# Human-Augment-Analytics/vectordb-retrieval

Hardware: AMD Instinct MI355X
Metric: QPS @ recall@10 (SIFT1M-shaped, 10k-query batch, k=10) (higher is better)
Workload: dtype i8 MFMA scan (i32 accumulate) + exact integer / f64 refine

## Files before the change

vectordb-retrieval_amd/csrc/scan_i8x16.hpp:

```cpp
#pragma once
#include "scan_i8.hpp"

namespace vdb {

__host__ __device__ inline int x16_row_in_span(int t, int rb, int m) { return (m >> 2) * 128 + t * 8 + rb * 4 + (m & 3); }

__device__ __forceinline__ int swap16(int v) { return __builtin_amdgcn_ds_swizzle(v, 0x401F); }

template <int KS2, int ST, int RING>
constexpr int scan_i8x16_lds_bytes() { return RING * (ST * 2 * KS2 * 64 * 16 + ST * 32 * 4); }

template <int N_MFMA, int N_VALU, int N_DS>
__device__ __forceinline__ void x16_gap_pattern() {
    constexpr int R = (N_VALU + N_DS + N_MFMA - 1) / N_MFMA;
    static_assert(N_DS <= N_MFMA && R >= 2, "one LDS read per gap");
#pragma unroll
    for (int i = 0; i < N_MFMA; ++i) {
        __builtin_amdgcn_sched_group_barrier(0x8, 1, 0);
        if (i < N_DS) {
            __builtin_amdgcn_sched_group_barrier(0x100, 1, 0);
            __builtin_amdgcn_sched_group_barrier(0x2, R - 1, 0);
        } else {
            __builtin_amdgcn_sched_group_barrier(0x2, R, 0);
        }
    }
}

template <int KS2, int ST, int CB, class StageIssue, class BiasStore, class FlushBin>
__device__ __forceinline__ void scan_i8x16_batch_loop(const unsigned char *smem, const int4v (&bq)[CB][KS2], int (&m1)[CB], int (&m2)[CB],
                                                      int nstages, int64_t span0, int lane, StageIssue &&stage_issue,
                                                      BiasStore &&stage_bias_store, FlushBin &&flush_bin) {
    constexpr int NV = 2 * KS2, kStageVec = ST * NV * 64, TPS = kTilesPerSpan, SPS = TPS / ST;
    constexpr int NM = 2 * KS2 * CB, NH = NM / 2;
    static_assert(ST % 2 == 0 && TPS % ST == 0, "tile parity must be static in the unrolled stage");
    const int g = lane >> 4;
    const unsigned id_hi = (g & 1) ? 16u : 0u;
    int4v acc[2][2][CB], fr[2][NV], cin[2][2];
    int q[CB];
#pragma unroll
    for (int rb = 0; rb < 2; ++rb)
#pragma unroll
        for (int cb = 0; cb < CB; ++cb)
#pragma unroll
            for (int r = 0; r < 4; ++r) acc[1][rb][cb][r] = (int)(kI8Inf >> 6);
    auto read_tile = [&](int p, const int4v *A, const int4v *B4, int t) {
#pragma unroll
        for (int v = 0; v < NV; ++v) fr[p][v] = A[(t * NV + v) * 64];
        cin[p][0] = B4[t * 8];
        cin[p][1] = B4[t * 8 + 1];
    };
    auto mfma_half = [&](int p, int half) {
#pragma unroll
        for (int m = half * NH; m < (half + 1) * NH; ++m) {
            const int ks = m / (2 * CB), rb = (m / CB) % 2, cb = m % CB;
            acc[p][rb][cb] = __builtin_amdgcn_mfma_i32_16x16x64_i8(fr[p][2 * ks + rb], bq[cb][ks], ks == 0 ? cin[p][rb] : acc[p][rb][cb], 0, 0, 0);
        }
    };
    auto min_trees = [&](int o) {
#pragma unroll
        for (int cb = 0; cb < CB; ++cb) {
            const int t1 = imin(imin(acc[o][0][cb][0], acc[o][0][cb][1]), acc[o][0][cb][2]);
            const int t2 = imin(imin(acc[o][0][cb][3], acc[o][1][cb][0]), acc[o][1][cb][1]);
            q[cb] = imin(imin(imin(acc[o][1][cb][2], acc[o][1][cb][3]), t1), t2);
        }
    };
    auto folds = [&](int t_bin) {
        const unsigned idv = (unsigned)__builtin_amdgcn_readfirstlane(t_bin) | id_hi;
#pragma unroll
        for (int cb = 0; cb < CB; ++cb) {
            const int v = (int)(((unsigned)q[cb] << 6) | idv);
            m2[cb] = imed3(m1[cb], m2[cb], v);
            m1[cb] = imin(m1[cb], v);
        }
    };
    for (int st = 0; st < nstages; ++st) {
        const int buf = st & 1;
        if (st + 1 < nstages) stage_issue(st + 1, buf ^ 1);
        const int4v *A = reinterpret_cast<const int4v *>(smem + buf * (kStageVec * 16)) + lane;
        const int4v *B4 = reinterpret_cast<const int4v *>(smem + 2 * kStageVec * 16 + buf * (ST * 32 * 4)) + g * 2;
        const int ts0 = (st % SPS) * ST;
        read_tile(0, A, B4, 0);
#pragma unroll
        for (int t = 0; t < ST; ++t) {
            const int p = t & 1, o = p ^ 1;
            __builtin_amdgcn_sched_barrier(0);
            mfma_half(p, 0);
            min_trees(o);
            x16_gap_pattern<NH, 4 * CB, 0>();
            __builtin_amdgcn_sched_barrier(0);
#pragma unroll
            for (int cb = 0; cb < CB; ++cb) asm volatile("" : "+v"(q[cb]));
            __builtin_amdgcn_sched_barrier(0);
            if (t + 1 < ST) read_tile(o, A, B4, t + 1);
            mfma_half(p, 1);
            folds((ts0 + t + TPS - 1) % TPS);
            x16_gap_pattern<NH, 3 * CB + 1, NV + 2>();
            __builtin_amdgcn_sched_barrier(0);
#pragma unroll
            for (int cb = 0; cb < CB; ++cb) asm volatile("" : "+v"(m1[cb]), "+v"(m2[cb]));
            if (t == 0 && st > 0 && ts0 == 0) flush_bin(span0 + st / SPS - 1);
        }
        __builtin_amdgcn_sched_barrier(0);
        if (st + 1 < nstages) stage_bias_store(buf ^ 1);
        __syncthreads();
    }
    min_trees((ST - 1) & 1);
    folds(TPS - 1);
    flush_bin(span0 + nstages / SPS - 1);
}

template <int KS2, int ST, int CB, int NWAVES = 8, int RING = 2, int AUX = 0>
__device__ __forceinline__ void scan_i8x16_body(const ScanI8Args &a, unsigned char *smem) {
    constexpr int NV = 2 * KS2;
    constexpr int NT = NWAVES * 64;
    constexpr int kStageVec = ST * NV * 64;
    constexpr int kBiasLoads = (ST * 32 + NT - 1) / NT;
    constexpr int TPS = kTilesPerSpan;
    constexpr int SPS = TPS / ST;
    constexpr int HC = CB / 2;
    constexpr int UNR = (ST * CB <= 16) ? ST : 1;
    static_assert(TPS % ST == 0 && ST >= 2 && CB % 2 == 0 && NWAVES <= 8, "bad geometry");
    static_assert(RING >= 2 && RING <= 8 && (RING == 2 || ST % 2 == 0), "bad ring");
    constexpr bool kDeep = RING > 2;
    static_assert(scan_i8x16_lds_bytes<KS2, ST, RING>() == RING * (kStageVec * 16 + ST * 32 * 4), "LDS size");
    const int mode = a.info->i8_mode;
    if (!mode) return;
    auto lds_a = [&](int buf) { return reinterpret_cast<int4v *>(smem + buf * (kStageVec * 16)); };
    auto lds_b = [&](int buf) { return reinterpret_cast<int *>(smem + RING * kStageVec * 16 + buf * (ST * 32 * 4)); };

    const int tid = threadIdx.x, lane = tid & 63;
    const int wave = __builtin_amdgcn_readfirstlane(tid >> 6);
    const int g = lane >> 4, h = g >> 1;
    const bool odd = (g & 1) != 0;
    const bool late = (NWAVES >= 2) && (wave >= NWAVES / 2);
    const int b = blockIdx.x;
    const int x = b & 7, jb = b >> 3;
    const int ci = jb / a.nqtiles, qt = jb - ci * a.nqtiles;
    const int chunk = x + 8 * ci;
    if (chunk >= a.nchunks) return;
    const int64_t q0 = (int64_t)qt * (NWAVES * 16 * CB) + wave * (16 * CB);
    const int64_t span0 = chunk_span0(chunk, a.spans_per_chunk, a.chunk_rem);
    int64_t span1 = chunk_span0(chunk + 1, a.spans_per_chunk, a.chunk_rem);
    if (span1 > a.nspans) span1 = a.nspans;
    const int64_t out_pitch = a.Qpad;
    const int64_t col0 = q0 + (odd ? 16 : 0) + (lane & 15);
    const int32_t *bias = a.bias8 + ((mode & 3) == 1 ? 0 : a.Npad);

    int4v bq[CB][KS2];
#pragma unroll
    for (int cb = 0; cb < CB; ++cb)
#pragma unroll
        for (int ks = 0; ks < KS2; ++ks) bq[cb][ks] = a.qpanels[((size_t)(q0 / 16 + cb) * KS2 + ks) * 64 + lane];
    const int nstages = (int)(span1 - span0) * SPS;
    const int INF = (int)kI8Inf;
    int m1[CB], m2[CB], M1[HC], M2[HC], Ms[HC];
#pragma unroll
    for (int cb = 0; cb < CB; ++cb) m1[cb] = m2[cb] = INF;
#pragma unroll
    for (int j = 0; j < HC; ++j) {
        M1[j] = M2[j] = INF;
        Ms[j] = 0;
    }

    constexpr int kPieces = kStageVec / 64;
    static_assert(kPieces % NWAVES == 0, "pieces must divide over the waves");
    constexpr int kBiasPieces = (ST / 2 + NWAVES - 1) / NWAVES;
    int stage_b[kBiasLoads];
    auto stage_issue = [&](int st, int buf) {
        const int64_t span = span0 + st / SPS;
        const int sq = st % SPS;
        const int4v *src = a.panels + ((size_t)(span * TPS + sq * ST) * NV) * 64;
        int4v *dst = lds_a(buf);
#pragma unroll
        for (int i = 0; i < kPieces / NWAVES; ++i) {
            const int p = wave + i * NWAVES;
            const int4v *gp = src + p * 64 + lane;
            __builtin_amdgcn_global_load_lds(
                reinterpret_cast<const __attribute__((address_space(1))) void *>(reinterpret_cast<uintptr_t>(gp)),
                reinterpret_cast<__attribute__((address_space(3))) void *>(
                    static_cast<uint32_t>(reinterpret_cast<uintptr_t>(dst + p * 64))),
                16, 0, AUX);
        }
        if (kDeep) {
#pragma unroll
            for (int i = 0; i < kBiasPieces; ++i) {
                const int j = (wave + i * NWAVES) % (ST / 2);
                const int t = 2 * j + (lane >> 5), gg = (lane >> 3) & 3, e = lane & 7;
                const int32_t *gp = bias + span * kSpanRows + gg * 128 + (sq * ST + t) * 8 + e;
                __builtin_amdgcn_global_load_lds(
                    reinterpret_cast<const __attribute__((address_space(1))) void *>(reinterpret_cast<uintptr_t>(gp)),
                    reinterpret_cast<__attribute__((address_space(3))) void *>(
                        static_cast<uint32_t>(reinterpret_cast<uintptr_t>(lds_b(buf) + j * 64))),
                    4, 0, 0);
            }
            return;
        }
#pragma unroll
        for (int i = 0; i < kBiasLoads; ++i) {
            const int e = tid + i * NT;
            if (e < ST * 32) {
                const int t = e >> 5, gg = (e >> 3) & 3, r = e & 7;
                stage_b[i] = bias[span * kSpanRows + gg * 128 + (sq * ST + t) * 8 + r];
            }
        }
    };
    auto stage_bias_store = [&](int buf) {
        if (kDeep) return;
#pragma unroll
        for (int i = 0; i < kBiasLoads; ++i)
            if (tid + i * NT < ST * 32) lds_b(buf)[tid + i * NT] = stage_b[i];
    };
    auto ring_issue = [&](int st) { stage_issue(st < nstages ? st : nstages - 1, st % RING); };
    auto ring_wait = [&]() {
        constexpr int kKeep = (RING - 2) * (kPieces / NWAVES + kBiasPieces);
        static_assert(kKeep < 64, "vmcnt is a 6-bit counter");
        asm volatile("s_waitcnt vmcnt(%0)" ::"n"(kKeep) : "memory");
        __builtin_amdgcn_s_barrier();
        asm volatile("" ::: "memory");
    };
    auto flush_bin = [&](int64_t span) {
        const size_t o = (size_t)(span * 2 + h) * out_pitch + col0;
#pragma unroll
        for (int j = 0; j < HC; ++j) {
            const int p1 = swap16(odd ? m1[2 * j] : m1[2 * j + 1]), p2 = swap16(odd ? m2[2 * j] : m2[2 * j + 1]);
            const int a1 = odd ? m1[2 * j + 1] : m1[2 * j], a2 = odd ? m2[2 * j + 1] : m2[2 * j];
            const int b1 = imin(a1, p1), b2 = imin(imax(a1, p1), imin(a2, p2));
            __builtin_nontemporal_store(__int_as_float(b1), a.bin_m1 + o + j * 32);
            __builtin_nontemporal_store(__int_as_float(b2), a.bin_m2 + o + j * 32);
            M2[j] = imin(imed3(M1[j], M2[j], b1), b2);
            if (b1 < M1[j]) Ms[j] = (int)span;
            M1[j] = imin(M1[j], b1);
        }
#pragma unroll
        for (int cb = 0; cb < CB; ++cb) m1[cb] = m2[cb] = INF;
    };

    if (kDeep) {
#pragma unroll
        for (int s = 0; s < RING - 1; ++s) ring_issue(s);
    } else {
        stage_issue(0, 0);
    }
    stage_bias_store(0);
    if (kDeep) ring_wait();
    else __syncthreads();

    if (a.nq_valid > 0 && q0 >= a.nq_valid) {
        for (int st = 0; st < nstages; ++st) {
            if (kDeep) {
                ring_issue(st + RING - 1);
                ring_wait();
                continue;
            }
            if (st + 1 < nstages) {
                stage_issue(st + 1, (st & 1) ^ 1);
                stage_bias_store((st & 1) ^ 1);
            }
            __syncthreads();
        }
        return;
    }

    if constexpr (NWAVES == 8 && RING == 2 && UNR == 1) {
        scan_i8x16_batch_loop<KS2, ST, CB>(smem, bq, m1, m2, nstages, span0, lane, stage_issue, stage_bias_store, flush_bin);
    } else {
    int4v fr[NV], cin[2], acc[2][CB];
    auto read_phase = [&](const int4v *A_tile, const int4v *c_tile) {
#pragma unroll
        for (int v = 0; v < NV; ++v) fr[v] = A_tile[v * 64 + lane];
        cin[0] = c_tile[0];
        cin[1] = c_tile[1];
    };
    auto mfma_phase = [&]() {
#pragma unroll
        for (int ks = 0; ks < KS2; ++ks)
#pragma unroll
            for (int rb = 0; rb < 2; ++rb)
#pragma unroll
                for (int cb = 0; cb < CB; ++cb)
                    acc[rb][cb] = __builtin_amdgcn_mfma_i32_16x16x64_i8(fr[2 * ks + rb], bq[cb][ks], ks == 0 ? cin[rb] : acc[rb][cb], 0, 0, 0);
    };
    const unsigned id_hi = odd ? 16u : 0u;
    auto select_phase = [&](int t_bin) {
        const unsigned idv = (unsigned)__builtin_amdgcn_readfirstlane(t_bin) | id_hi;
#pragma unroll
        for (int cb = 0; cb < CB; ++cb) {
            const int t1 = imin(imin(acc[0][cb][0], acc[0][cb][1]), acc[0][cb][2]);
            const int t2 = imin(imin(acc[0][cb][3], acc[1][cb][0]), acc[1][cb][1]);
            const int q = imin(imin(imin(acc[1][cb][2], acc[1][cb][3]), t1), t2);
            const int v = (int)(((unsigned)q << 6) | idv);
            m2[cb] = imed3(m1[cb], m2[cb], v);
            m1[cb] = imin(m1[cb], v);
        }
    };
    if (a.prio == 1 && late) __builtin_amdgcn_s_setprio(1);
    else if (a.prio == 2 && !late) __builtin_amdgcn_s_setprio(1);
    if (!late) {
        for (int st = 0; st < nstages; ++st) {
            const int buf = kDeep ? st % RING : st & 1;
            if (kDeep) ring_issue(st + RING - 1);
            else if (st + 1 < nstages) stage_issue(st + 1, buf ^ 1);
            const int4v *A = lds_a(buf);
            const int4v *B4 = reinterpret_cast<const int4v *>(lds_b(buf)) + g * 2;
            const int ts0 = (st % SPS) * ST;
            read_phase(A, B4);
#pragma unroll UNR
            for (int t = 0; t < ST; ++t) {
                __builtin_amdgcn_sched_barrier(0);
                mfma_phase();
                __builtin_amdgcn_sched_barrier(0);
                if (t + 1 < ST) read_phase(A + (t + 1) * NV * 64, B4 + (t + 1) * 8);
                select_phase(ts0 + t);
            }
            __builtin_amdgcn_sched_barrier(0);
            if (ts0 + ST == TPS) flush_bin(span0 + st / SPS);
            if (!kDeep && st + 1 < nstages) stage_bias_store(buf ^ 1);
            if (kDeep) ring_wait();
            else __syncthreads();
        }
    } else {
#pragma unroll
        for (int rb = 0; rb < 2; ++rb)
#pragma unroll
            for (int cb = 0; cb < CB; ++cb)
#pragma unroll
                for (int r = 0; r < 4; ++r) acc[rb][cb][r] = (int)(kI8Inf >> 6);
        for (int st = 0; st < nstages; ++st) {
            const int buf = kDeep ? st % RING : st & 1;
            if (kDeep) ring_issue(st + RING - 1);
            else if (st + 1 < nstages) stage_issue(st + 1, buf ^ 1);
            const int4v *A = lds_a(buf);
            const int4v *B4 = reinterpret_cast<const int4v *>(lds_b(buf)) + g * 2;
            const int ts0 = (st % SPS) * ST;
#pragma unroll UNR
            for (int t = 0; t < ST; ++t) {
                __builtin_amdgcn_sched_barrier(0);
                read_phase(A + t * NV * 64, B4 + t * 8);
                select_phase((ts0 + t + TPS - 1) % TPS);
                if (t == 0 && st > 0 && ts0 == 0) flush_bin(span0 + st / SPS - 1);
                __builtin_amdgcn_sched_barrier(0);
                mfma_phase();
            }
            __builtin_amdgcn_sched_barrier(0);
            if (!kDeep && st + 1 < nstages) stage_bias_store(buf ^ 1);
            if (kDeep) ring_wait();
            else __syncthreads();
        }
        select_phase(TPS - 1);
        flush_bin(span1 - 1);
    }
    }

    const size_t so = (size_t)(chunk * 2 + h) * a.Qpad + col0;
#pragma unroll
    for (int j = 0; j < HC; ++j) {
        a.sb_m1[so + j * 32] = __int_as_float(M1[j]);
        a.sb_m2[so + j * 32] = __int_as_float(M2[j]);
        a.sb_span[so + j * 32] = Ms[j];
    }
}

template <int KS2, int ST, int CB, int NWAVES = 8, int RING = 2, int AUX = 0>
__global__ __launch_bounds__(NWAVES * 64, (NWAVES >= 4 ? 2 : 1)) void scan_i8x16_kernel(ScanI8Args a) {
    __shared__ __attribute__((aligned(16))) unsigned char smem[scan_i8x16_lds_bytes<KS2, ST, RING>()];
    scan_i8x16_body<KS2, ST, CB, NWAVES, RING, AUX>(a, smem);
}

}
```

Before: 11.72 million.

## Move stage barrier inside last tile and prefetch next stage's first tile

Restructures the double-buffered stage loop so the bias store and workgroup barrier happen inside the last unrolled tile. This lets the first tile of the next buffer be read from LDS before the final MFMA half, and the global issue for stage st+2 runs after the barrier. The goal is to hide the per-stage barrier and tile-read latency behind MFMA work. It also replaces the ds_swizzle-based bin flush with permlane16_swap, and mirrors the new barrier protocol in the idle-wave path. The risk is a race on buffer reuse if the waitcnt and barrier placement is wrong.

```diff
diff --git a/vectordb-retrieval_amd/csrc/scan_i8x16.hpp b/vectordb-retrieval_amd/csrc/scan_i8x16.hpp
--- a/vectordb-retrieval_amd/csrc/scan_i8x16.hpp
+++ b/vectordb-retrieval_amd/csrc/scan_i8x16.hpp
@@ -24,6 +24,12 @@
             __builtin_amdgcn_sched_group_barrier(0x2, R, 0);
         }
     }
+}
+
+__device__ __forceinline__ void x16_stage_barrier() {
+    asm volatile("s_waitcnt vmcnt(0) lgkmcnt(0)" ::: "memory");
+    __builtin_amdgcn_s_barrier();
+    asm volatile("" ::: "memory");
 }
 
 template <int KS2, int ST, int CB, class StageIssue, class BiasStore, class FlushBin>
@@ -73,16 +79,18 @@
             m1[cb] = imin(m1[cb], v);
         }
     };
+    auto lds_frag = [&](int buf) { return reinterpret_cast<const int4v *>(smem + buf * (kStageVec * 16)) + lane; };
+    auto lds_bias = [&](int buf) { return reinterpret_cast<const int4v *>(smem + 2 * kStageVec * 16 + buf * (ST * 32 * 4)) + g * 2; };
+    if (nstages > 1) stage_issue(1, 1);
+    read_tile(0, lds_frag(0), lds_bias(0), 0);
     for (int st = 0; st < nstages; ++st) {
         const int buf = st & 1;
-        if (st + 1 < nstages) stage_issue(st + 1, buf ^ 1);
-        const int4v *A = reinterpret_cast<const int4v *>(smem + buf * (kStageVec * 16)) + lane;
-        const int4v *B4 = reinterpret_cast<const int4v *>(smem + 2 * kStageVec * 16 + buf * (ST * 32 * 4)) + g * 2;
+        const int4v *A = lds_frag(buf), *B4 = lds_bias(buf);
         const int ts0 = (st % SPS) * ST;
-        read_tile(0, A, B4, 0);
 #pragma unroll
         for (int t = 0; t < ST; ++t) {
             const int p = t & 1, o = p ^ 1;
+            if (t == ST - 1) stage_bias_store(buf ^ 1);
             __builtin_amdgcn_sched_barrier(0);
             mfma_half(p, 0);
             min_trees(o);
@@ -90,8 +98,13 @@
             __builtin_amdgcn_sched_barrier(0);
 #pragma unroll
             for (int cb = 0; cb < CB; ++cb) asm volatile("" : "+v"(q[cb]));
-            __builtin_amdgcn_sched_barrier(0);
-            if (t + 1 < ST) read_tile(o, A, B4, t + 1);
+            if (t == ST - 1) {
+                x16_stage_barrier();
+                A = lds_frag(buf ^ 1);
+                B4 = lds_bias(buf ^ 1);
+            }
+            __builtin_amdgcn_sched_barrier(0);
+            read_tile(o, A, B4, (t + 1) % ST);
             mfma_half(p, 1);
             folds((ts0 + t + TPS - 1) % TPS);
             x16_gap_pattern<NH, 3 * CB + 1, NV + 2>();
@@ -101,8 +114,7 @@
             if (t == 0 && st > 0 && ts0 == 0) flush_bin(span0 + st / SPS - 1);
         }
         __builtin_amdgcn_sched_barrier(0);
-        if (st + 1 < nstages) stage_bias_store(buf ^ 1);
-        __syncthreads();
+        if (st + 2 < nstages) stage_issue(st + 2, buf);
     }
     min_trees((ST - 1) & 1);
     folds(TPS - 1);
@@ -235,6 +247,24 @@
         for (int cb = 0; cb < CB; ++cb) m1[cb] = m2[cb] = INF;
     };
 
+    auto flush_bin_swap = [&](int64_t span) {
+        const size_t o = (size_t)(span * 2 + h) * out_pitch + col0;
+#pragma unroll
+        for (int j = 0; j < HC; ++j) {
+            const auto s1 = __builtin_amdgcn_permlane16_swap((unsigned)m1[2 * j], (unsigned)m1[2 * j + 1], false, false);
+            const auto s2 = __builtin_amdgcn_permlane16_swap((unsigned)m2[2 * j], (unsigned)m2[2 * j + 1], false, false);
+            const int a1 = (int)s1[0], p1 = (int)s1[1];
+            const int b1 = imin(a1, p1), b2 = imin(imax(a1, p1), imin((int)s2[0], (int)s2[1]));
+            __builtin_nontemporal_store(__int_as_float(b1), a.bin_m1 + o + j * 32);
+            __builtin_nontemporal_store(__int_as_float(b2), a.bin_m2 + o + j * 32);
+            M2[j] = imin(imed3(M1[j], M2[j], b1), b2);
+            if (b1 < M1[j]) Ms[j] = (int)span;
+            M1[j] = imin(M1[j], b1);
+        }
+#pragma unroll
+        for (int cb = 0; cb < CB; ++cb) m1[cb] = m2[cb] = INF;
+    };
+
     if (kDeep) {
 #pragma unroll
         for (int s = 0; s < RING - 1; ++s) ring_issue(s);
@@ -245,7 +275,17 @@
     if (kDeep) ring_wait();
     else __syncthreads();
 
+    constexpr bool kBatch = NWAVES == 8 && RING == 2 && UNR == 1;
     if (a.nq_valid > 0 && q0 >= a.nq_valid) {
+        if constexpr (kBatch) {
+            if (nstages > 1) stage_issue(1, 1);
+            for (int st = 0; st < nstages; ++st) {
+                stage_bias_store((st & 1) ^ 1);
+                x16_stage_barrier();
+                if (st + 2 < nstages) stage_issue(st + 2, st & 1);
+            }
+            return;
+        }
         for (int st = 0; st < nstages; ++st) {
             if (kDeep) {
                 ring_issue(st + RING - 1);
@@ -261,8 +301,8 @@
         return;
     }
 
-    if constexpr (NWAVES == 8 && RING == 2 && UNR == 1) {
-        scan_i8x16_batch_loop<KS2, ST, CB>(smem, bq, m1, m2, nstages, span0, lane, stage_issue, stage_bias_store, flush_bin);
+    if constexpr (kBatch) {
+        scan_i8x16_batch_loop<KS2, ST, CB>(smem, bq, m1, m2, nstages, span0, lane, stage_issue, stage_bias_store, flush_bin_swap);
     } else {
     int4v fr[NV], cin[2], acc[2][CB];
     auto read_phase = [&](const int4v *A_tile, const int4v *c_tile) {
```

New measurement: 11.81 million (median of 6 runs). About the same (+0.8%).
